# tangle-network/zk-SaaS

Hardware: AMD Instinct MI355X
Metric: Groth16 proofs/sec (SHA-256 circuit) (higher is better)
Workload: dtype u32 limbs (256-bit Montgomery); 1 GPU; BASELINE configs[3]: full distributed Groth16 on the SHA-256 circuit, BN254, l=2, n=8 parties on one GPU, all 12 masks sampled and applied (sha256.rs:226-291); masks=True, constraints=30006, wires=29823, domain=32768, len_a=14911, len_w=14911, len_u=16384, parties=8, packing_factor=2, fixed_base_tables=True

## Files before the change

zk-saas_amd/csrc/engine_groth16.inc.hpp:

```cpp

  int king3(const Fr* in, const zk_groth16_masks* mk, int first, int log_m, int inverse, const void* g, int scale,
            int rearrange, uint64_t seed, Fr* out, size_t per, hipStream_t st) {
    const Fr* U = nullptr;
    int rc = umat_for(nullptr, n, &U);
    if (rc) return rc;
    KingBatch<Fr> kb{};
    kb.stride = per;
    bool any = false, all = true;
    for (int k = 0; k < 3; k++) {
      kb.in_mask[k] = mk ? (const Fr*)mk->fft_in[first + k] : nullptr;
      kb.out_mask[k] = mk ? (const Fr*)mk->fft_out[first + k] : nullptr;
      any = any || kb.in_mask[k];
      all = all && kb.in_mask[k];
    }
    if (any == all)
      return king_dispatch_batch(in, kb, 3, n, log_m, inverse, U, g, scale, rearrange, seed, out, false, st);
    for (int k = 0; k < 3; k++) {
      rc = king_dispatch(in + k * per, kb.in_mask[k], n, log_m, inverse, U, g, scale, rearrange, seed + k,
                         out + k * per, kb.out_mask[k], false, st);
      if (rc) return rc;
    }
    return ZK_OK;
  }
  int circom_h(const void* qa, const void* qb, const void* qc, int log_m, const zk_groth16_masks* mk, uint64_t seed,
// ... 386 lines not shown
    ProveJob* J = &j;
    const size_t cstride = crs->len_a;
    const Fr* cf = msm_.coef_d_ + first;
    MsmGate gate{};
    const bool gated = j.gate_sorts = (full || gate_sorts) && log_m >= h_first_log_m_;
    j.sorted_cnt.store(0, std::memory_order_relaxed);
    if (gated) {
      gate.sorted_cnt = &j.sorted_cnt;
      gate.wait_sorted = j.ev_role;
      gate.n_wait_sorted = gate.sorted_need = 4;
    }
    auto role_gate = [&](MsmRole role) {
      MsmGate g = gate;
      if (g.n_wait_sorted) g.sorted_ev = J->ev_role[role];
      return g;
    };
    bool hu_done = false;
    if (full && gated) {
      hipError_t he = j.hshare.ensure((size_t)n * Lc * sizeof(Fr));
      if (he != hipSuccess) return hip_fail(he, "h share buffer");
      rc = circom_h_ws(qa, qb, qc, log_m, mk, seed, j.hshare.p, j.hwork, streams_[5]);
      if (rc) return rc;
      rc = msm_.template launch_t<Fq_>(this, j.ws0 + ROLE_U, crs->u_d, j.hshare.p, (size_t)n * crs->len_u,
                                      msm_.coef_d_, crs->len_u, streams_[5], &j.msm[ROLE_U], nullptr, u_gate(j));
      if (rc) return rc;
      hu_done = true;
    }
    msm_task<Fq2_>(j, ROLE_V, crs->v_d, nullptr, a_share, nullptr, (size_t)count * cstride, cf, cstride, streams_[2],
                   role_gate(ROLE_V), nullptr, [this, J](const P2* res) { take_V(*J, res); });
    const void* hd = j.pt.r_zero ? nullptr : crs->h_d;
    msm_task<Fq_>(j, ROLE_SH, crs->s_d, hd, a_share, nullptr, (size_t)count * cstride, cf, cstride, streams_[0],
                  role_gate(ROLE_SH), nullptr, [this, J, hd](const P1* res) { take_SH(*J, res, hd != nullptr); });
    msm_task<Fq_>(j, ROLE_W, crs->w_d, nullptr, ax_share, nullptr, (size_t)count * crs->len_w, cf, crs->len_w, streams_[3],
                  role_gate(ROLE_W), nullptr, [this, J](const P1* res) { take_W(*J, res); });
    if (!(full && !hu_done)) submit_host_terms(&j.pt, j.fut);
    if (full && !hu_done) {
      host_span(PROF_HOST_SUBMIT);
      hipStream_t hs = streams_[5];
      hipError_t he = j.hshare.ensure((size_t)n * Lc * sizeof(Fr));
      if (he != hipSuccess) return hip_fail(he, "h share buffer");
      rc = circom_h_ws(qa, qb, qc, log_m, mk, seed, j.hshare.p, j.hwork, hs);
      if (rc) return rc;
      host_span(PROF_HOST_H);
      rc = msm_.template launch_t<Fq_>(this, j.ws0 + ROLE_U, crs->u_d, j.hshare.p, (size_t)n * crs->len_u,
                                      msm_.coef_d_, crs->len_u, hs, &j.msm[ROLE_U]);
      if (rc) return rc;
      submit_host_terms(&j.pt, j.fut);
      host_span(PROF_HOST_U);
    }
    return ZK_OK;
  }

  void submit_host_terms(ProofTerms* J, std::vector<std::future<void>>& fut) {
    const bool full = J->full;
    const int first = J->first, count = J->count;
    if (full) {
      fut.push_back(pool_->submit([J]() {
        P1 d1 = aff1(J->crs.delta_g1);
        J->rN = host_scalar_mul<FrP, Fq_>(d1, J->r);
        J->s_cA = host_scalar_mul<FrP, Fq_>(xyzz_add_ni(xyzz_add_ni(aff1(J->crs.a_query0), J->rN), aff1(J->crs.alpha_g1)), J->s);
      }));
      fut.push_back(pool_->submit([J]() {
        P1 d1 = aff1(J->crs.delta_g1);
        J->sK = host_scalar_mul<FrP, Fq_>(d1, J->s);
        J->r_cB1 = host_scalar_mul<FrP, Fq_>(xyzz_add_ni(xyzz_add_ni(aff1(J->crs.b_g1_query0), J->sK), aff1(J->crs.beta_g1)), J->r);
      }));
      fut.push_back(pool_->submit([J]() { J->rsM = host_scalar_mul<FrP, Fq_>(aff1(J->crs.delta_g1), J->r * J->s); }));
      fut.push_back(pool_->submit([J]() { J->sK2 = host_scalar_mul<FrP, Fq2_>(aff2(J->crs.delta_g2), J->s); }));
// ... 10 lines not shown
            J->in1[k] = msm_.template mask_term<Fq_>(im, first, count);
            if (k == 0 && J->full) J->s_in0 = host_scalar_mul<FrP, Fq_>(J->in1[0], J->s);
            if (k == 1 && J->full) J->r_in1 = host_scalar_mul<FrP, Fq_>(J->in1[1], J->r);
          }
        }));
      }
      if (full)
        for (int p = 0; p < n; p++) {
          if (mk->msm_out[0])
            fut.push_back(pool_->submit([J, p]() {
              J->s_om0[p] = host_scalar_mul<FrP, Fq_>(jacobian_to_xyzz(((const Jacobian<Fq_>*)J->mk.msm_out[0])[p]), J->s);
            }));
          if (mk->msm_out[1] && !J->r_zero)
            fut.push_back(pool_->submit([J, p]() {
              J->r_om1[p] = host_scalar_mul<FrP, Fq_>(jacobian_to_xyzz(((const Jacobian<Fq_>*)J->mk.msm_out[1])[p]), J->r);
            }));
        }
    }
  }

  int prove_launch_u(ProveJob& j, const void* h_share, hipStream_t st) {
    const ProofTerms& t = j.pt;
    return msm_.template launch_t<Fq_>(this, j.ws0 + ROLE_U, t.crs.u_d, h_share, (size_t)t.count * t.crs.len_u,
                                      msm_.coef_d_ + t.first, t.crs.len_u, st, &j.msm[ROLE_U], nullptr, u_gate(j));
  }

  int prove_end(ProveJob& j, void* pi_a, void* pi_b, void* pi_c) {
    const char* who = "zk_groth16_wait";
    const auto t0 = std::chrono::steady_clock::now();
    int rc = drain_or_wedge(j, who);
    if (rc) return rc;
    bool early_ok = !j.pt.err.code;
    for (int e : j.rc) early_ok = early_ok && !e;
    std::vector<P1> c_part(early_ok ? n : 0);
    if (early_ok) assemble_job(j.pt, j.pt.sums(), pi_a, pi_b, pi_c, c_part.data());
    if (prof.on && job_slot(j, ROLE_U).busy) (void)event_wait(job_slot(j, ROLE_U).ev);
    const auto t2 = std::chrono::steady_clock::now();
    struct HostSpans {
      Profiler& pr;
      std::chrono::steady_clock::time_point a, b;
      ~HostSpans() {
        if (!pr.on) return;
        pr.host_add(PROF_HOST_WAIT, std::chrono::duration<double, std::milli>(b - a).count());
        pr.host_add(PROF_HOST_TAIL, std::chrono::duration<double, std::milli>(std::chrono::steady_clock::now() - b).count());
      }
    } spans{prof, t0, t2};
    rc = join(j, who);
// ... 335 lines not shown
```

zk-saas_amd/csrc/engine_points.inc.hpp:

```cpp

  int msm(int group, const void* bases, size_t nb, const void* scalars, size_t ns, void* out,
          hipStream_t st) override {
    if (nb != ns) {
      return fail(ZK_ERR_GENERIC, std::to_string(nb < ns ? nb : ns));
    }
    return msm_.run(this, group, bases, scalars, nb, out, st);
  }
  int d_msm(int group, const void* bases, const void* scalars, size_t len, const void* in_mask, const void* out_mask,
            void* out, hipStream_t st) override {
    return msm_.d_msm(this, group, bases, scalars, len, in_mask, out_mask, out, st);
  }

  static constexpr size_t BASE_MUL_WIDE_FROM = (size_t)1 << 19;
  template <class Fld>
  int base_mul_t(const void* base_affine, const void* scalars, size_t len, void* out_affine, hipStream_t st) {
    if (!len) return ZK_OK;
    if (!base_affine || !scalars || !out_affine) return fail(ZK_ERR_BAD_INPUT, "null pointer");
    const int nwin = (FrP::BITS + 7) / 8;
    std::string key((const char*)base_affine, sizeof(Affine<Fld>));
    Affine<Fld>* table = nullptr;
    {
      std::lock_guard<std::mutex> lk(mu_);
      auto it = base_tables_.find(key);
      if (it != base_tables_.end()) table = (Affine<Fld>*)it->second;
// ... 258 lines not shown
      if (value != 0 && (value < 8 || value > 22)) return fail(ZK_ERR_BAD_INPUT, "msm_table_c_g2 must be 0 (by length) or in 8..22");
      msm_.table_c_g2 = (int)value;
      return ZK_OK;
    }
    if (!strcmp(name, "wait_deadline_ms")) {
      if (value < 0 || value > 86400000) return fail(ZK_ERR_BAD_INPUT, "wait_deadline_ms must be in 0..86400000");
      wait_deadline_ms.store(value, std::memory_order_relaxed);
      return ZK_OK;
    }
    if (!strcmp(name, "host_threads")) {
      if (value < 0 || value > 256) return fail(ZK_ERR_BAD_INPUT, "host_threads must be in 0..256");
      if (value && value < 4) return fail(ZK_ERR_BAD_INPUT, "host_threads must be 0 (automatic) or at least 4");
      std::lock_guard<std::mutex> lk(mu_);
      if (streams_ready_) return fail(ZK_ERR_BAD_INPUT, "host_threads must be set before the first proof");
      host_threads_ = (int)value;
      return ZK_OK;
    }
    if (!strcmp(name, "msm_c") || !strcmp(name, "msm_c_g2")) {
      if (value != 0 && (value < 2 || value > 20)) return fail(ZK_ERR_BAD_INPUT, "msm_c must be 0 or in 2..20");
      if (name[5] == 0) msm_.c_g1 = msm_.c_g2 = (int)value;
      else msm_.c_g2 = (int)value;
      return ZK_OK;
    }
    if (!strcmp(name, "h_first_log_m")) {
      if (value < 1 || value > 64) return fail(ZK_ERR_BAD_INPUT, "h_first_log_m must be in 1..64");
      h_first_log_m_ = (int)value;
      return ZK_OK;
    }
    return fail(ZK_ERR_BAD_INPUT, "unknown option");
  }
  int msm_plan(int group, size_t len, int* plan) override {
    if (!plan || (group != ZK_G1 && group != ZK_G2)) return fail(ZK_ERR_BAD_INPUT, "bad argument");
    if (group == ZK_G2 && !Cfg::HAS_G2) return fail(ZK_ERR_BAD_INPUT, "G2 is not available for this curve");
    msm_.plan(len, group == ZK_G2, plan);
    return ZK_OK;
  }
  int group_add(int group, const void* a, const void* b, void* out) override {
    using Fq = Fp<typename Cfg::FqP>;
    using Fq2 = Fp2<typename Cfg::FqP>;
    if (!a || !b || !out) return fail(ZK_ERR_BAD_INPUT, "null pointer");
    if (group == ZK_G1) {
      Jacobian<Fq> x, y;
      memcpy(&x, a, sizeof(x));
      memcpy(&y, b, sizeof(y));
      Jacobian<Fq> o = xyzz_to_jacobian(xyzz_add_ni(jacobian_to_xyzz(x), jacobian_to_xyzz(y)));
      memcpy(out, &o, sizeof(o));
// ... 398 lines not shown
```

zk-saas_amd/csrc/msm.hpp:

```cpp
#pragma once
#include <algorithm>
#include <atomic>
#include <cstdio>
#include <cstdlib>
#include <future>
#include <map>
#include <memory>
#include <mutex>
#include <type_traits>
#include <vector>

#include "ec.hpp"
#include "engine.hpp"
#include "msm_plan.hpp"
#include "ntt.hpp"
#include "quad.hpp"

namespace zk {
#if defined(__HIPCC__)

enum MsmRole { ROLE_SH, ROLE_W, ROLE_V, ROLE_U, NROLES };
constexpr const char* ROLE_NAME[NROLES] = {"S+H", "W", "V", "U"};
constexpr int NJOBS = 2;
constexpr int NBATCH = 3;
// ... 1057 lines not shown
      for (uint32_t j = (uint32_t)vl; j < S; j += FIN_THREADS / 4) acc = qadd(acc, qload(hpart + vb + j, q), q);
      acc = wg_quad_sum(acc, sh, vl, q, FIN_THREADS / 4);
      if (vl == 0) qstore(buckets + heavy[2 + 2 * h], q, acc);
      __syncthreads();
    }
    return;
  }
  const uint32_t T = msm_range_len(offsets[nkeys], nlanes, tmin, cap);
  for (size_t k = (size_t)blockIdx.x * (FIN_THREADS / 4) + (threadIdx.x >> 2); k < nkeys;
       k += (size_t)fin_wgs * (FIN_THREADS / 4)) {
    const uint32_t o0 = offsets[k], o1 = offsets[k + 1];
    if (o0 == o1) {
      qstore(buckets + k, q, qidentity<Fld>(q));
      continue;
    }
    const uint32_t l0 = o0 / T, l1 = (o1 - 1) / T;
    if (l1 == l0 || l1 - l0 > FIN_SEQ) continue;
    Fld acc = qload(tail + l0, q);
    for (uint32_t l = l0 + 1; l <= l1; l++) acc = qadd(acc, qload(head + l, q), q);
    qstore(buckets + k, q, acc);
  }
}

template <class Fld>
__global__ __launch_bounds__(QUAD_THREADS, 2) void msm_reduce_a_kernel(const XYZZ<Fld>* __restrict__ buckets0, uint32_t B,
                                                                   int lo_bits, int nvl, XYZZ<Fld>* __restrict__ out0) {
  __builtin_amdgcn_s_setprio(3);
  extern __shared__ uint4 smem_red[];
  XYZZ<Fld>* sh = reinterpret_cast<XYZZ<Fld>*>(smem_red);
  const uint32_t LO = 1u << lo_bits, HI = B >> lo_bits;
  const uint32_t ngroups = HI + 1 + LO;
  const XYZZ<Fld>* __restrict__ wb = buckets0 + (size_t)blockIdx.y * B;
  const int q = threadIdx.x & 3, vl = threadIdx.x >> 2;
  const uint32_t g = blockIdx.x * (uint32_t)((int)blockDim.x / 4 / nvl) + (uint32_t)(vl / nvl);
  const uint32_t sub = (uint32_t)(vl & (nvl - 1));
  Fld acc = qidentity<Fld>(q);
  if (g <= HI) {
    for (uint32_t lo = sub; lo < LO; lo += (uint32_t)nvl) {
      uint32_t k = g * LO + lo;
      if (k >= 1 && k <= B) acc = qadd(acc, qload(wb + (k - 1), q), q);
    }
  } else if (g < ngroups) {
    const uint32_t lo = g - HI - 1;
    for (uint32_t hi = sub; hi <= HI; hi += (uint32_t)nvl) {
      uint32_t k = hi * LO + lo;
      if (k >= 1 && k <= B) acc = qadd(acc, qload(wb + (k - 1), q), q);
// ... 106 lines not shown
  const void* p[16] = {nullptr};
};

struct MsmPending {
  MsmFoldGeo fold;
  MsmSlot* slot = nullptr;
};

struct MsmGate {
  hipEvent_t sorted_ev = nullptr;
  std::atomic<int>* sorted_cnt = nullptr;
  const hipEvent_t* wait_sorted = nullptr;
  int n_wait_sorted = 0, sorted_need = 0;
  hipEvent_t wait_ev = nullptr;
  std::atomic<int>* wait_flag = nullptr;
  hipEvent_t signal_ev = nullptr;
  std::atomic<int>* signal_flag = nullptr;
};

struct MsmTuning {
  size_t bigsort_min;
  MsmGate gate;
  int c_force = 0;
};

template <class FrP, class Fld>
int msm_launch(IEngine* eng, MsmSlot& slot, const MsmTuning& tune, const void* bases, const void* bases2,
               const void* scalars, size_t npts, const Fp<FrP>* coef_d, size_t part_len, hipStream_t st,
               MsmPending* out, const MsmBatchArg* batch = nullptr);
template <class FrP, class Fld>
int pack_points_split_launch(IEngine* eng, const void* points, size_t nchunks, int n, const uint8_t* dig, int jlen,
                             const void* beta , void* shares, hipStream_t st);
template <class FrP, class Fld>
int base_mul_split_launch(IEngine* eng, const void* scalars, size_t len, const void* table, int nwin, int wb, void* out,
                          hipStream_t st);
template <class FrP, class Fld>
int msm_table_launch(IEngine* eng, const void* bases, size_t len, int c, int nwin, int wide, void* table,
                     hipStream_t st);

template <class Fld>
int msm_fold_batch(IEngine* eng, MsmPending& p, XYZZ<Fld>* results, int nvec) {
  const MsmFoldGeo& f = p.fold;
  const int batch = f.batch;
  for (int i = 0; i < nvec * batch; i++) results[i] = XYZZ<Fld>::identity();
  if (!p.slot) return ZK_OK;
  hipError_t he = p.slot->wait(eng);
// ... 124 lines not shown
  for (int nib = FrP::N * 8 - 1; nib >= 0; nib--) {
    for (int i = 0; i < 4; i++) acc = xyzz_dbl_ni(acc);
    for (int p = 0; p < np; p++) {
      uint32_t d = (k[p].v[nib / 8] >> (4 * (nib % 8))) & 15u;
      if (d) acc = xyzz_add_ni(acc, tab[(size_t)p * 15 + d - 1]);
    }
  }
  return acc;
}

template <class Cfg>
class MsmRunner {
 public:
  using FrP = typename Cfg::FrP;
  using Fr = Fp<FrP>;
  using Fq = Fp<typename Cfg::FqP>;
  using Fq2 = Fp2<typename Cfg::FqP>;

  void plan(size_t npts, bool g2, int* out) const {
    MsmPlanIn in;
    in.scalar_bits = FrP::BITS, in.scalar_bytes = (int)sizeof(Fr), in.coord_bytes = (int)(g2 ? sizeof(Fq2) : sizeof(Fq));
    in.g2 = g2, in.acc_waves = g2 ? SPLIT_WAVES<typename Cfg::FqP> : ACC_WAVES<Fq>;
    in.npts = npts, in.c_force = g2 ? c_g2 : c_g1, in.bigsort_min = bigsort_min;
    msm_plan_of(in, out);
  }
  int c_g1 = 0, c_g2 = 0;

  template <class Fld>
  int launch_t(IEngine* eng, int ws, const void* bases, const void* scalars, size_t npts, const Fr* coef_d,
               size_t part_len, hipStream_t st, MsmPending* pend, const void* bases2 = nullptr, MsmGate gate = MsmGate{},
               const MsmBatchArg* batch = nullptr) {
    if (ws < 0 || ws >= MSM_WS) return eng->fail(ZK_ERR_BAD_INPUT, "bad msm workspace slot");
    if (slots_[ws].busy) return eng->fail(ZK_ERR_GENERIC, "msm workspace slot still in flight");
    MsmTuning tune{bigsort_min, gate, IsExtField<Fld>::value ? c_g2 : c_g1};
    int rc = msm_launch<FrP, Fld>(eng, slots_[ws], tune, bases, bases2, scalars, npts, coef_d, part_len, st, pend,
                                  batch);
    if (rc) (void)slots_[ws].wait(eng);
    return rc;
  }
  template <class Fld, class Host>
  int run_t(IEngine* eng, int sid, const void* bases, const void* scalars, size_t npts, const Fr* coef_d,
            size_t part_len, hipStream_t st, XYZZ<Fld>* out, Host&& host, const MsmBatchArg* batch = nullptr) {
    int rc = eng->check_wedged();
    if (rc) return rc;
    std::unique_lock<std::mutex> lk(standalone_mu_, std::defer_lock);
    if (sid < 0) lk.lock();
    MsmPending pend;
    rc = launch_t<Fld>(eng, sid < 0 ? WS_STANDALONE : ws_dist(sid), bases, scalars, npts, coef_d, part_len, st, &pend,
                       nullptr, MsmGate{}, batch);
    if (!rc) {
      host();
      rc = msm_fold_batch<Fld>(eng, pend, out, 1);
    }
    if (rc && pend.slot && pend.slot->busy) {
      Status keep = eng->last;
      return eng->wedge(keep.msg);
    }
// ... 182 lines not shown
```

zk-saas_amd/csrc/msm_impl.hpp:

```cpp
#pragma once
#include "msm.hpp"
#include "pack_split.hpp"

namespace zk {

#define MSM_HIP(x)                                           \
  do {                                                       \
    hipError_t _e = (x);                                     \
    if (_e != hipSuccess) return eng->hip_fail(_e, #x);      \
  } while (0)
#ifdef ZK_MSM_DEBUG_SYNC
#define MSM_STAGE(name)                                                          \
  do {                                                                           \
    hipError_t _e = hipStreamSynchronize(st);                                    \
    fprintf(stderr, "[zk msm] %s done (%s) npts=%zu c=%d nwin=%d\n", name,       \
            hipGetErrorString(_e), pl.npts, pl.win.c, pl.win.nwin);              \
    if (_e != hipSuccess) return eng->hip_fail(_e, name);                        \
  } while (0)
#else
#define MSM_STAGE(name) do { } while (0)
#endif

template <class Fr, class KF>
struct MsmViews {
// ... 113 lines not shown
    msm_accumulate_split_kernel<typename BaseParams<Fld>::type><<<dim3((nlanes + 31) / 32, NB), dim3(128), 0, st>>>(
        bases, bases2, v.sorted, v.offsets, nkeys, nlanes, pl.tmin, pl.cap, v.buckets, v.edge, v.heavy, v.k0, pl.ys);
  } else {
    msm_accumulate_kernel<KF><<<dim3((nlanes + 127) / 128, NB), dim3(128), 0, st>>>(
        (const Affine<KF>*)bases, (const Affine<KF>*)bases2, v.sorted, v.offsets, nkeys, nlanes, pl.tmin, pl.cap, v.buckets,
        v.edge, v.heavy, v.k0, pl.ys, 0);
  }
  if (gate.signal_ev) {
    MSM_HIP(hipEventRecord(gate.signal_ev, st));
    if (gate.signal_flag) gate.signal_flag->store(1, std::memory_order_release);
  }
  return ZK_OK;
}

template <class Fr, class Fld, class KF>
int msm_stage_reduce(IEngine* eng, const MsmPlan& pl, const MsmViews<Fr, KF>& v, hipStream_t st) {
  constexpr bool G2FLD = IsExtField<Fld>::value;
  const unsigned NB = pl.vectors, nsets = (unsigned)pl.nsets;
  const uint32_t nkeys = (uint32_t)pl.nkeys, nlanes = pl.nlanes, tmin = pl.tmin, cap = pl.cap;
  const size_t ys = pl.ys;
  ProfScope ps_(eng->prof, G2FLD ? PROF_MSM_REDUCE_G2 : PROF_MSM_REDUCE, st, (double)pl.nkeys * NB);
  const int qt = quad_threads(pl.batch > 1), qvl = qt / 4;
  const size_t quad_lds = (size_t)qvl * sizeof(XYZZ<Fld>);
  msm_heavy_kernel<KF><<<dim3(2048, NB), dim3(64), (size_t)16 * sizeof(XYZZ<Fld>), st>>>(v.edge, nlanes, tmin, cap, v.offsets, nkeys,
                                                                    v.buckets, v.heavy, v.hpart, pl.vcap, ys);
  MSM_STAGE("heavy buckets");
  {
    const size_t fin_wgs = std::min<size_t>((pl.nkeys + FIN_THREADS / 4 - 1) / (FIN_THREADS / 4), 8192);
    const unsigned fin_extra = 256;
    msm_finalize_kernel<KF><<<dim3((unsigned)fin_wgs + fin_extra, NB), dim3(FIN_THREADS),
                              (size_t)(FIN_THREADS / 4) * sizeof(XYZZ<Fld>), st>>>(
        v.edge, nlanes, tmin, cap, v.offsets, nkeys, v.buckets, v.heavy, v.hpart, pl.vcap, (uint32_t)fin_wgs, ys);
  }
  MSM_STAGE("finalize");
  const size_t tot_groups = (size_t)pl.red_groups * NB * nsets;
  const size_t tot_slices = (size_t)pl.nslices * NB * nsets;
  const size_t cap_quads = (size_t)1024 * (G2FLD ? 2 : 3) * 16;
  auto pick_nvl = [&](size_t groups) {
    int n = qvl;
    while (n > 4 && groups * (size_t)n > cap_quads) n >>= 1;
    return n;
  };
  const int nvl_a = pick_nvl(tot_groups), nvl_b = pick_nvl(tot_slices);
  const unsigned gpw_a = (unsigned)(qvl / nvl_a), gpw_b = (unsigned)(qvl / nvl_b);
  msm_reduce_a_kernel<KF><<<dim3((pl.red_groups + gpw_a - 1) / gpw_a, NB * nsets), dim3((unsigned)qt), quad_lds, st>>>(
      v.buckets, pl.B, pl.lo_bits, nvl_a, v.rc);
  msm_reduce_b_kernel<KF><<<dim3(((unsigned)pl.nslices + gpw_b - 1) / gpw_b, NB * nsets), dim3((unsigned)qt), quad_lds, st>>>(
      v.rc, pl.B, pl.lo_bits, nvl_b, v.out,
      v.offsets + nkeys, ys, pl.nsorts, v.stats);
  return ZK_OK;
}

template <class FrP, class Fld>
int msm_launch(IEngine* eng, MsmSlot& slot, const MsmTuning& tune, const void* bases, const void* bases2,
               const void* scalars, size_t npts, const Fp<FrP>* coef_d, size_t part_len, hipStream_t st,
               MsmPending* pend, const MsmBatchArg* ba) {
  using Fr = Fp<FrP>;
// ... 2 lines not shown
  static_assert(sizeof(XYZZ<Fld>) == 4 * sizeof(Fld), "the plan sizes XYZZ points as four coordinates");
  constexpr bool G2FLD = IsExtField<Fld>::value;
  *pend = MsmPending{};
  const unsigned NB = bases2 ? 2u : 1u;
  const void* const bases_in = bases;
  const void* const bases2_in = bases2;
  size_t toff = 0, toff2 = 0;
  std::shared_ptr<const MsmTable> tab = TableRegistry::inst().find(bases, npts, sizeof(Affine<Fld>), FrP::BITS, &toff), tab2;
  if (tab && NB == 2) {
    tab2 = TableRegistry::inst().find(bases2, npts, sizeof(Affine<Fld>), FrP::BITS, &toff2);
    if (!tab2 || tab2->len != tab->len || toff2 != toff || tab2->c != tab->c) tab = nullptr;
    else bases2 = tab2->data;
  }
  if (tab) bases = tab->data;
  MsmPlanIn in;
  in.scalar_bits = FrP::BITS, in.scalar_bytes = (int)sizeof(Fr), in.coord_bytes = (int)sizeof(Fld), in.g2 = G2FLD;
  if constexpr (G2FLD) in.acc_waves = SPLIT_WAVES<typename BaseParams<Fld>::type>;
  else in.acc_waves = ACC_WAVES<Fld>;
  in.npts = npts, in.batch = ba ? (size_t)ba->nb : 1, in.vectors = (int)NB;
  if (tab) {
    in.tab_c = tab->c, in.tab_len = tab->len, in.tab_off = toff;
    in.tab_no_identity = !tab->any_identity && (NB == 1 || !tab2->any_identity);
  }
  in.c_force = tune.c_force, in.bigsort_min = tune.bigsort_min;
  const MsmPlan pl = msm_plan(in);
  if (pl.err) return eng->fail(ZK_ERR_BAD_INPUT, pl.err);
  pend->fold = pl.fold;
  if (npts == 0) return ZK_OK;
  hipError_t he = slot.ws.ensure(pl.ws_bytes);
  if (he != hipSuccess) return eng->hip_fail(he, "msm workspace");
  he = slot.ensure_pinned(pl.pinned_bytes);
  if (he != hipSuccess) return eng->hip_fail(he, "msm pinned buffer");
  if (!slot.ev) {
    he = hipEventCreateWithFlags(&slot.ev, hipEventDisableTiming);
    if (he != hipSuccess) return eng->hip_fail(he, "msm event");
  }
  slot.busy = true;
  slot.tab = tab;
  slot.tab2 = tab2;
  pend->slot = &slot;
  struct RecordOnExit {
    MsmSlot& s;
    hipStream_t st;
    bool done = false;
    ~RecordOnExit() {
      if (!done) (void)hipEventRecord(s.ev, st);
    }
// ... 87 lines not shown
```

zk-saas_amd/csrc/msm_plan.hpp:

```cpp
#pragma once
#include <algorithm>
#include <cstddef>
#include <cstdint>

namespace zk {

constexpr size_t MSM_RANGE_MIN = 20, MSM_RANGE = 64;
constexpr size_t MSM_RANGE_MIN_G2 = 16, MSM_RANGE_G2 = 64;
constexpr uint32_t FIN_SEQ = 16;
constexpr int MSM_MAXB = 16;

constexpr int BIG_HI = 8;
constexpr int BIG_MAX_BINS = 8192;
constexpr int BIG_THREADS = 256;
constexpr int BIG_PTS_PER_THREAD = 8;
constexpr int BIG_EPT = 16;
constexpr size_t BIG_LDS_MAX = 156 * 1024;
inline int msm_big_hi(size_t nsets) {
  int hi = BIG_HI;
  while (hi > 0 && (nsets << hi) > (size_t)BIG_MAX_BINS) hi--;
  return hi;
}
constexpr size_t msm_bins_words(size_t nbins) { return 3 * nbins + 2; }

constexpr int ISCAN_THREADS = 256;
constexpr int ISCAN_PER = 8;
constexpr int ISCAN_BLOCK = ISCAN_THREADS * ISCAN_PER;

inline size_t msm_heavy_cap(size_t nlanes) { return nlanes / FIN_SEQ + 8; }
inline size_t msm_heavy_vcap(size_t nlanes) { return nlanes / FIN_SEQ + nlanes / 256 + 8; }

struct MsmWindows {
// ... 9 lines not shown
  int width(int w) const { return w < wide ? c : c - 1; }
  int start(int w) const { return w * (c - 1) + std::min(w, wide); }
};

inline int msm_pick_c(int scalar_bits, size_t npts, int c_force = 0) {
  if (c_force >= 2 && c_force <= 20) return c_force;
  int best = 4;
  double best_cost = 1e300;
  for (int c = 4; c <= 20; c++) {
    int nwin = (scalar_bits + c) / c;
    int ceff = (scalar_bits + nwin) / nwin;
    double cost = (double)nwin * ((double)npts + (ceff > 17 ? 10.0 : 4.0) * (double)((size_t)1 << (ceff - 1)));
    if (cost <= best_cost) {
      best_cost = cost;
      best = c;
    }
  }
  return best;
}

struct MsmLanes {
  uint32_t nlanes, tmin, cap;
};
inline MsmLanes msm_pick_lanes(size_t max_entries, int waves, bool pair, int lanes_per_range = 0) {
  if (!lanes_per_range) lanes_per_range = pair ? 2 : 1;
  const size_t cap = (size_t)1024 * waves * (64 / lanes_per_range);
  const size_t lo = pair ? MSM_RANGE_MIN_G2 : MSM_RANGE_MIN;
  const size_t hi = pair ? MSM_RANGE_G2 : MSM_RANGE;
  size_t t = std::min(hi, std::max(lo, (size_t)((double)max_entries / (2.4 * (double)cap))));
  size_t nl = std::max<size_t>(1, (max_entries + t - 1) / t);
  if (max_entries >= cap * t && max_entries < 2 * cap * t && (max_entries + 2 * cap - 1) / (2 * cap) >= 12)
    nl = std::max(nl, 2 * cap);
  return MsmLanes{(uint32_t)nl, (uint32_t)t, (uint32_t)cap};
}

inline int table_c_auto(size_t len, bool g2) {
  if (g2) return len < ((size_t)1 << 20) ? 15 : 19;
  return len <= ((size_t)1 << 17) ? 15 : len < ((size_t)1 << 19) ? 16 : len < ((size_t)1 << 22) ? 18 : 20;
}

struct MsmFoldGeo {
  MsmWindows win;
  int kwin = 0;
  int lo_bits = 0;
  bool tabbed = false;
  int batch = 1;
  int nb = 1;
  int nsorts = 1;
  size_t stats_off = 0;
  size_t offered = 0;
  bool g2 = false;
};

struct MsmPlanIn {
  int scalar_bits = 0, scalar_bytes = 0;
  int coord_bytes = 0;
  bool g2 = false;
  int acc_waves = 0;
  size_t npts = 0, batch = 1;
  int vectors = 1;
  int tab_c = 0;
  size_t tab_len = 0, tab_off = 0;
  bool tab_no_identity = false;
  int c_force = 0;
  size_t bigsort_min = 0;
};

enum MsmRegionId {
  R_COUNTS, R_HEAVY, R_BINS, R_CURSOR, R_OFFSETS, R_BT, R_SORTED, R_K0, R_CANON, R_TMP, R_TMP_LO, R_TCNT,
  R_EDGE, R_BUCKETS, R_HPART, R_RC,
  R_COUNT,
  R_SORT_END = R_EDGE
};
struct MsmRegion {
  size_t off = 0, bytes = 0;
};

struct MsmPlan {
  const char* err = nullptr;
  size_t npts = 0, batch = 1;
  unsigned vectors = 1;
  MsmWindows win;
  uint32_t B = 0;
  bool tabbed = false;
  int kwin = 0;
  size_t nsets = 0, nkeys = 0;
  size_t max_sorted = 0;
  uint32_t pre_stride = 0, pre_off = 0;
  uint32_t nlanes = 0, tmin = 0, cap = 0;
  uint32_t vcap = 0;
  int lo_bits = 0;
  uint32_t red_groups = 0;
  int nslices = 0;
  size_t iscan_blocks = 0;
  bool no_identity = false;
  unsigned nsorts = 1;
  bool big = false;
  bool large = false;
  int sthr = 0, ppt = 0;
  int sort_hi = 0, sort_lo = 0;
  int idx_bits = 0;
  bool wide_fmt = false;
  size_t nbl = 0;
  size_t nbins_tot = 0;
  size_t stage_cap = 0, tile_pts = 0, tiles_big = 0;
  int wgroup = 0;
  bool use_tcnt = false;
  int hist_ppt = 0;
  size_t hist_lds = 0, scatter_lds = 0, binsort_lds = 0;
  MsmRegion r[R_COUNT];
  size_t sort_region = 0;
  size_t ys = 0;
  size_t ws_bytes = 0;
// ... 3 lines not shown
  MsmFoldGeo fold;
};

inline MsmPlan msm_plan(const MsmPlanIn& in) {
  MsmPlan p;
  const size_t npts = in.npts, batch = in.batch;
  const unsigned NB = in.vectors == 2 ? 2u : 1u;
  const bool tab = in.tab_c != 0;
  p.npts = npts, p.batch = batch, p.vectors = NB, p.tabbed = tab;
  if (batch < 1 || batch > (size_t)MSM_MAXB) {
    p.err = "bad msm batch";
    return p;
  }
  p.fold.batch = (int)batch;
  const MsmWindows win = MsmWindows::of(in.scalar_bits, tab ? in.tab_c : msm_pick_c(in.scalar_bits, npts ? npts : 1, in.c_force));
  const int c = win.c, nwin = win.nwin;
  p.win = win;
  p.B = 1u << (c - 1);
  const uint32_t B = p.B;
  const int kwin = p.kwin = tab ? 1 : nwin;
  const size_t nsets = p.nsets = batch * (size_t)kwin;
  const size_t nkeys = p.nkeys = nsets * B;
  const size_t max_sorted = p.max_sorted = npts * batch * nwin;
  const MsmLanes ml = msm_pick_lanes(max_sorted, in.acc_waves, in.g2, in.g2 ? 4 : 0);
  const uint32_t nlanes = p.nlanes = ml.nlanes;
  p.tmin = ml.tmin, p.cap = ml.cap;
  if (npts * batch >= ((size_t)1 << 31)) p.err = "msm too large";
  else if (max_sorted >= ((size_t)1 << 32)) p.err = "msm too large (points x windows >= 2^32)";
  if (p.err || !npts) return p;
  p.pre_stride = tab ? (uint32_t)in.tab_len : 0u, p.pre_off = tab ? (uint32_t)in.tab_off : 0u;
  p.vcap = (uint32_t)msm_heavy_vcap(nlanes);
  const int lo_bits = p.lo_bits = c / 2;
  p.red_groups = (B >> lo_bits) + 1 + (1u << lo_bits);
  p.nslices = c;
  p.iscan_blocks = (nkeys + ISCAN_BLOCK - 1) / ISCAN_BLOCK;
  p.no_identity = tab && in.tab_no_identity;
  const unsigned NS = p.nsorts = (NB == 2 && !p.no_identity) ? 2u : 1u;

  constexpr size_t large_min = (size_t)4 << 20;
  const bool large = p.large = npts * batch >= large_min;
  const int sthr = p.sthr = large ? 1024 : 256;
  int ppt = large ? BIG_PTS_PER_THREAD : 16;
  if (!large)
    while (ppt > 1 && ((npts + (size_t)sthr * ppt - 1) / ((size_t)sthr * ppt)) * batch < 1024) ppt >>= 1;
  const size_t stage_max = 16384;
  if (large && tab)
    while (ppt > 1 && (size_t)nwin * sthr * ppt > stage_max) ppt >>= 1;
  p.ppt = ppt;
  int sort_hi = std::min(msm_big_hi(nsets), std::max(1, c - 1 - 7));
  if (large) {
    auto lg = [](size_t v) { int l = 0; while (((size_t)1 << (l + 1)) <= v) l++; return l; };
    const int tp_eff = lg((size_t)sthr * ppt * (tab ? nwin : 1)), ch = lg((size_t)sthr * BIG_EPT);
    sort_hi = (c - 1 + tp_eff - ch + 1) / 2;
    if (sort_hi > c - 2) sort_hi = c - 2;
// ... 19 lines not shown
  const size_t tile_pts = p.tile_pts = (size_t)sthr * ppt;
  const bool big = p.big = npts * batch >= in.bigsort_min && sort_hi >= 1 && sort_lo >= 1 && sort_lo <= 12 &&
                           (nsets << sort_hi) <= (size_t)BIG_MAX_BINS &&
                           (large ? stage_cap >= (tab ? (size_t)nwin * tile_pts : tile_pts) : 8 * nbl <= BIG_LDS_MAX);
  p.wgroup = tab ? nwin : (int)std::min<size_t>((size_t)nwin, std::max<size_t>(1, stage_cap / tile_pts));
  const size_t nbins_tot = p.nbins_tot = nsets << sort_hi;
  p.tiles_big = ((npts + tile_pts - 1) / tile_pts) * batch;
  p.use_tcnt = big && large && tile_pts % BIG_THREADS == 0 && tile_pts < 65536;
  if (big) {
    p.hist_ppt = p.use_tcnt ? (int)(tile_pts / BIG_THREADS) : ppt;
    p.hist_lds = (nbins_tot + BIG_THREADS / 64) * 4;
    p.scatter_lds = large ? (2 * nbl + (size_t)(sthr / 64)) * 4 + stage_cap * (wide_fmt ? 8 : 6) : 2 * nbl * 4;
    p.binsort_lds = (2 * ((size_t)1 << sort_lo) + 1 + (size_t)(sthr / 64)) * 4 + (large ? (size_t)sthr * BIG_EPT * 6 : 0);
  }

  size_t off = 0;
  auto take = [&](MsmRegionId id, size_t bytes) {
    p.r[id].off = off;
    p.r[id].bytes = bytes;
    off += (bytes + 255) & ~(size_t)255;
  };
  const size_t xyzz = 4 * (size_t)in.coord_bytes;
  take(R_COUNTS, nkeys * 4);
  take(R_HEAVY, msm_heavy_cap(nlanes) * 8 + 16);
  take(R_BINS, big ? msm_bins_words(nbins_tot) * 4 : 0);
  p.zero_off = big ? p.r[R_HEAVY].off : p.r[R_COUNTS].off;
  p.zero_bytes = big ? p.r[R_BINS].off + (nbins_tot + 1) * 4 - p.zero_off : p.r[R_HEAVY].off + 16 - p.zero_off;
  take(R_CURSOR, nkeys * 4);
  take(R_OFFSETS, (nkeys + 1) * 4);
  take(R_BT, p.iscan_blocks * 4);
  take(R_SORTED, max_sorted * 4);
  take(R_K0, (size_t)nlanes * 4);
  take(R_CANON, npts * batch * (size_t)in.scalar_bytes);
  if (big) {
    take(R_TMP, max_sorted * 4);
    if (wide_fmt) take(R_TMP_LO, max_sorted * 2);
    if (p.use_tcnt) take(R_TCNT, p.tiles_big * nbl * 2);
  }
  p.sort_region = off;
  p.ys = NS == 2 ? p.sort_region : 0;
  off = p.sort_region * NS;
  take(R_EDGE, NB * 2 * (size_t)nlanes * xyzz);
  take(R_BUCKETS, NB * nkeys * xyzz);
  take(R_HPART, NB * (size_t)p.vcap * xyzz);
  take(R_RC, NB * nsets * p.red_groups * xyzz);
  p.ws_bytes = off;
  p.out_bytes = NB * nsets * p.nslices * xyzz;
  p.pinned_bytes = p.out_bytes + 64;

  p.fold.win = win;
// ... 22 lines not shown
```

zk-saas_amd/csrc/quad.hpp:

```cpp
#pragma once
#include "ec.hpp"
#include "ntt.hpp"

namespace zk {
#if defined(__HIPCC__)

template <int P0, int P1, int P2, int P3>
ZK_D uint32_t qperm_u32(uint32_t v) {
  return (uint32_t)__builtin_amdgcn_mov_dpp((int)v, P0 | (P1 << 2) | (P2 << 4) | (P3 << 6), 0xf, 0xf, true);
}
template <int P0, int P1, int P2, int P3, class P>
ZK_D Fp<P> qperm(const Fp<P>& v) {
  Fp<P> r;
#pragma unroll
  for (int i = 0; i < P::N; i++) r.v[i] = qperm_u32<P0, P1, P2, P3>(v.v[i]);
  return r;
}
template <int P0, int P1, int P2, int P3, class P, bool I>
ZK_D Fp2T<P, I> qperm(const Fp2T<P, I>& v) {
  return {qperm<P0, P1, P2, P3>(v.c0), qperm<P0, P1, P2, P3>(v.c1)};
}
template <class P>
ZK_D Fp<P> qsel(bool a, const Fp<P>& x, const Fp<P>& y) {
  Fp<P> r;
#pragma unroll
  for (int i = 0; i < P::N; i++) r.v[i] = a ? x.v[i] : y.v[i];
  return r;
}
template <class P, bool I>
ZK_D Fp2T<P, I> qsel(bool a, const Fp2T<P, I>& x, const Fp2T<P, I>& y) {
  return {qsel(a, x.c0, y.c0), qsel(a, x.c1, y.c1)};
}

template <class Fld>
ZK_D Fld qidentity(int q) {
  return q < 2 ? Fld::one() : Fld::zero();
}
template <class Fld>
ZK_D Fld qload(const XYZZ<Fld>* p, int q) {
  return load_elem(reinterpret_cast<const Fld*>(p) + q);
}
template <class Fld>
ZK_D void qstore(XYZZ<Fld>* p, int q, const Fld& c) {
  store_elem(reinterpret_cast<Fld*>(p) + q, c);
}

template <class Fld>
ZK_D Fld qadd(const Fld& ca, const Fld& cb, int q) {
  const bool even = (q & 1) == 0;
  const bool za = qperm<2, 2, 2, 2>(ca).is_zero();
  const bool zb = qperm<2, 2, 2, 2>(cb).is_zero();
  Fld A = qsel(even, qperm<0, 0, 1, 1>(ca), qperm<0, 0, 1, 1>(cb));
  Fld B = qsel(even, qperm<2, 2, 3, 3>(cb), qperm<2, 2, 3, 3>(ca));
  const Fld m1 = A * B;
  const Fld d = qperm<1, 1, 3, 3>(m1) - qperm<0, 0, 2, 2>(m1);
  const bool pz = qperm<0, 0, 0, 0>(d).is_zero();
  const bool rz = qperm<2, 2, 2, 2>(d).is_zero();
  const bool D = pz && rz && !za && !zb;
  const Fld cu = qsel(q == 1, ca.dbl(), ca);
  A = qsel(D, cu, qsel(even, d, qperm<0, 2, 2, 3>(ca)));
  B = qsel(D, cu, qsel(even, d, qperm<0, 2, 2, 3>(cb)));
  const Fld m2 = A * B;
  const Fld XX = qperm<0, 0, 0, 0>(m2);
  const Fld M = XX.dbl() + XX;
  A = qsel(D, qsel(q == 3, M, cu), qsel(q == 2, qperm<0, 1, 1, 3>(m2), qsel(q == 1, d, m1)));
  B = qsel(D, qsel(q == 3, M, qperm<1, 1, 1, 1>(m2)), XX);
  const Fld m3 = A * B;
// ... 189 lines not shown
```

Before: 636.1 proofs/s.

## Fuse heavy-bucket and finalize MSM stages into one tail kernel for U MSM

Adds a fused msm_tail_kernel that handles heavy buckets (split across workgroups, with an atomic ticket so the last one combines the partials) and light-bucket finalization in a single launch. Light buckets are combined with a DPP row-rotate tree over groups of four lanes. The fused kernel is enabled for the U (h) MSM launches, which sit at the end of the dependency chain, and can be forced for all MSMs through a new 'msm_tail_latency' option. It targets a kernel launch and a serial stage on the critical path, at the cost of extra ticket memory that must be zeroed and a more complex synchronisation scheme.

```diff
diff --git a/zk-saas_amd/csrc/engine_groth16.inc.hpp b/zk-saas_amd/csrc/engine_groth16.inc.hpp
--- a/zk-saas_amd/csrc/engine_groth16.inc.hpp
+++ b/zk-saas_amd/csrc/engine_groth16.inc.hpp
@@ -432,7 +432,8 @@
       rc = circom_h_ws(qa, qb, qc, log_m, mk, seed, j.hshare.p, j.hwork, streams_[5]);
       if (rc) return rc;
       rc = msm_.template launch_t<Fq_>(this, j.ws0 + ROLE_U, crs->u_d, j.hshare.p, (size_t)n * crs->len_u,
-                                      msm_.coef_d_, crs->len_u, streams_[5], &j.msm[ROLE_U], nullptr, u_gate(j));
+                                      msm_.coef_d_, crs->len_u, streams_[5], &j.msm[ROLE_U], nullptr, u_gate(j), nullptr,
+                                      true );
       if (rc) return rc;
       hu_done = true;
     }
@@ -453,7 +454,8 @@
       if (rc) return rc;
       host_span(PROF_HOST_H);
       rc = msm_.template launch_t<Fq_>(this, j.ws0 + ROLE_U, crs->u_d, j.hshare.p, (size_t)n * crs->len_u,
-                                      msm_.coef_d_, crs->len_u, hs, &j.msm[ROLE_U]);
+                                      msm_.coef_d_, crs->len_u, hs, &j.msm[ROLE_U], nullptr, MsmGate{}, nullptr,
+                                      true );
       if (rc) return rc;
       submit_host_terms(&j.pt, j.fut);
       host_span(PROF_HOST_U);
@@ -510,7 +512,8 @@
   int prove_launch_u(ProveJob& j, const void* h_share, hipStream_t st) {
     const ProofTerms& t = j.pt;
     return msm_.template launch_t<Fq_>(this, j.ws0 + ROLE_U, t.crs.u_d, h_share, (size_t)t.count * t.crs.len_u,
-                                      msm_.coef_d_ + t.first, t.crs.len_u, st, &j.msm[ROLE_U], nullptr, u_gate(j));
+                                      msm_.coef_d_ + t.first, t.crs.len_u, st, &j.msm[ROLE_U], nullptr, u_gate(j), nullptr,
+                                      true );
   }
 
   int prove_end(ProveJob& j, void* pi_a, void* pi_b, void* pi_c) {
diff --git a/zk-saas_amd/csrc/engine_points.inc.hpp b/zk-saas_amd/csrc/engine_points.inc.hpp
--- a/zk-saas_amd/csrc/engine_points.inc.hpp
+++ b/zk-saas_amd/csrc/engine_points.inc.hpp
@@ -304,6 +304,11 @@
       else msm_.c_g2 = (int)value;
       return ZK_OK;
     }
+    if (!strcmp(name, "msm_tail_latency")) {
+      if (value != 0 && value != 1) return fail(ZK_ERR_BAD_INPUT, "msm_tail_latency must be 0 or 1");
+      msm_.tail_latency = (int)value;
+      return ZK_OK;
+    }
     if (!strcmp(name, "h_first_log_m")) {
       if (value < 1 || value > 64) return fail(ZK_ERR_BAD_INPUT, "h_first_log_m must be in 1..64");
       h_first_log_m_ = (int)value;
diff --git a/zk-saas_amd/csrc/msm.hpp b/zk-saas_amd/csrc/msm.hpp
--- a/zk-saas_amd/csrc/msm.hpp
+++ b/zk-saas_amd/csrc/msm.hpp
@@ -1103,6 +1103,103 @@
   }
 }
 
+constexpr uint32_t FIN_TREE_PRE = 2;
+template <class Fld>
+constexpr int TAIL_WAVES = sizeof(Fld) <= 32 ? 4 : sizeof(Fld) <= 48 ? 3 : 2;
+template <class Fld>
+__global__ __launch_bounds__(FIN_THREADS, TAIL_WAVES<Fld>) void msm_tail_kernel(const XYZZ<Fld>* __restrict__ edge0, uint32_t nlanes,
+                                                               uint32_t tmin, uint32_t cap,
+                                                               const uint32_t* __restrict__ offsets, uint32_t nkeys,
+                                                               XYZZ<Fld>* __restrict__ buckets0, uint32_t* __restrict__ heavy,
+                                                               XYZZ<Fld>* __restrict__ hpart0, uint32_t vcap, uint32_t hcap,
+                                                               uint32_t heavy_wgs, size_t ys) {
+  static_assert(FIN_TREE_G == 4 && FIN_THREADS == 64, "a group is one DPP row: 16 lanes, four per wave");
+  __builtin_amdgcn_s_setprio(3);
+  ZK_YSHIFT(offsets);
+  const XYZZ<Fld>* __restrict__ head = edge0 + (size_t)blockIdx.y * 2 * nlanes;
+  const XYZZ<Fld>* __restrict__ tail = head + nlanes;
+  XYZZ<Fld>* __restrict__ buckets = buckets0 + (size_t)blockIdx.y * nkeys;
+  const int q = threadIdx.x & 3, vl = threadIdx.x >> 2;
+  if (blockIdx.x < heavy_wgs) {
+    ZK_YSHIFT(heavy);
+    const uint32_t nh = heavy[1], V = heavy[0];
+    if (blockIdx.x >= V) return;
+    uint32_t* ticket = heavy + 2 + 2 * (size_t)hcap + (ys ? 0 : (size_t)blockIdx.y * hcap);
+    XYZZ<Fld>* hpart = hpart0 + (size_t)blockIdx.y * vcap;
+    extern __shared__ uint4 smem_fin[];
+    XYZZ<Fld>* sh = reinterpret_cast<XYZZ<Fld>*>(smem_fin);
+    __shared__ uint32_t last_sh;
+    constexpr int nq = FIN_THREADS / 4;
+    const uint32_t T = msm_range_len(offsets[nkeys], nlanes, tmin, cap);
+    for (uint32_t v = blockIdx.x; v < V; v += heavy_wgs) {
+      uint32_t lo = 0, hi = nh;
+      while (hi - lo > 1) {
+        const uint32_t mid = (lo + hi) >> 1;
+        if (heavy[3 + 2 * mid] <= v) lo = mid;
+        else hi = mid;
+      }
+      const uint32_t kh = heavy[2 + 2 * lo], vb = heavy[3 + 2 * lo];
+      const uint32_t S = (lo + 1 < nh ? heavy[3 + 2 * (lo + 1)] : V) - vb, s = v - vb;
+      const uint32_t o0 = offsets[kh], o1 = offsets[kh + 1];
+      const uint32_t l0 = o0 / T, l1 = (o1 - 1) / T;
+      const uint32_t chunk = (l1 - l0 + S - 1) / S;
+      const uint32_t first = l0 + 1 + s * chunk, last = first + chunk - 1 < l1 ? first + chunk - 1 : l1;
+      Fld acc = (s == 0 && vl == 0) ? qload(tail + l0, q) : qidentity<Fld>(q);
+      for (uint32_t l = first + (uint32_t)vl; l <= last; l += (uint32_t)nq) acc = qadd(acc, qload(head + l, q), q);
+      acc = wg_quad_sum(acc, sh, vl, q, nq);
+      if (vl == 0) qstore(S == 1 ? buckets + kh : hpart + v, q, acc);
+      if (S > 1) {
+        __builtin_amdgcn_fence(__ATOMIC_RELEASE, "agent");
+        __syncthreads();
+        if (threadIdx.x == 0)
+          last_sh = __hip_atomic_fetch_add(ticket + lo, 1u, __ATOMIC_ACQ_REL, __HIP_MEMORY_SCOPE_AGENT) == S - 1 ? 1u : 0u;
+        __syncthreads();
+        if (last_sh) {
+          __builtin_amdgcn_fence(__ATOMIC_ACQUIRE, "agent");
+          Fld t = qidentity<Fld>(q);
+          for (uint32_t j = (uint32_t)vl; j < S; j += (uint32_t)nq) t = qadd(t, qload_agent(hpart + vb + j, q), q);
+          t = wg_quad_sum(t, sh, vl, q, nq);
+          if (vl == 0) qstore(buckets + kh, q, t);
+        }
+      }
+      __syncthreads();
+    }
+    return;
+  }
+  const uint32_t T = msm_range_len(offsets[nkeys], nlanes, tmin, cap);
+  const uint32_t fin_wgs = gridDim.x - heavy_wgs;
+  constexpr uint32_t GPW = FIN_THREADS / 4 / FIN_TREE_G;
+  const uint32_t j = (uint32_t)vl & (FIN_TREE_G - 1);
+  for (size_t k = (size_t)(blockIdx.x - heavy_wgs) * GPW + (uint32_t)vl / FIN_TREE_G; k < nkeys; k += (size_t)fin_wgs * GPW) {
+    const uint32_t o0 = offsets[k], o1 = offsets[k + 1];
+    if (o0 == o1) {
+      if (j == 0) qstore(buckets + k, q, qidentity<Fld>(q));
+      continue;
+    }
+    const uint32_t l0 = o0 / T, l1 = (o1 - 1) / T;
+    if (l1 == l0 || l1 - l0 > FIN_SEQ) continue;
+    const uint32_t n = l1 - l0 + 1;
+    auto slot = [&](uint32_t i) {
+      const uint32_t idx = j + i * FIN_TREE_G, ic = idx < n ? idx : n - 1;
+      return qsel(idx < n, qload(ic ? head + l0 + ic : tail + l0, q), qidentity<Fld>(q));
+    };
+    Fld p[FIN_TREE_PRE];
+#pragma unroll
+    for (uint32_t i = 0; i < FIN_TREE_PRE; i++) p[i] = slot(i);
+    const uint32_t trips = (n + FIN_TREE_G - 1) / FIN_TREE_G;
+    Fld acc = p[0];
+#pragma unroll 1
+    for (uint32_t it = 1; it < trips + 2; it++) {
+      const Fld other = qsel(it < trips, p[1], qsel(it == trips, qrow_ror<8>(acc), qrow_ror<4>(acc)));
+#pragma unroll
+      for (uint32_t i = 1; i + 1 < FIN_TREE_PRE; i++) p[i] = p[i + 1];
+      p[FIN_TREE_PRE - 1] = slot(it + FIN_TREE_PRE - 1);
+      acc = qadd(acc, other, q);
+    }
+    if (j == 0) qstore(buckets + k, q, acc);
+  }
+}
+
 template <class Fld>
 __global__ __launch_bounds__(QUAD_THREADS, 2) void msm_reduce_a_kernel(const XYZZ<Fld>* __restrict__ buckets0, uint32_t B,
                                                                    int lo_bits, int nvl, XYZZ<Fld>* __restrict__ out0) {
@@ -1255,6 +1352,7 @@
   size_t bigsort_min;
   MsmGate gate;
   int c_force = 0;
+  bool chain_end = false;
 };
 
 template <class FrP, class Fld>
@@ -1425,17 +1523,19 @@
     in.scalar_bits = FrP::BITS, in.scalar_bytes = (int)sizeof(Fr), in.coord_bytes = (int)(g2 ? sizeof(Fq2) : sizeof(Fq));
     in.g2 = g2, in.acc_waves = g2 ? SPLIT_WAVES<typename Cfg::FqP> : ACC_WAVES<Fq>;
     in.npts = npts, in.c_force = g2 ? c_g2 : c_g1, in.bigsort_min = bigsort_min;
+    in.chain_end = tail_latency != 0;
     msm_plan_of(in, out);
   }
   int c_g1 = 0, c_g2 = 0;
+  int tail_latency = 0;
 
   template <class Fld>
   int launch_t(IEngine* eng, int ws, const void* bases, const void* scalars, size_t npts, const Fr* coef_d,
                size_t part_len, hipStream_t st, MsmPending* pend, const void* bases2 = nullptr, MsmGate gate = MsmGate{},
-               const MsmBatchArg* batch = nullptr) {
+               const MsmBatchArg* batch = nullptr, bool chain_end = false) {
     if (ws < 0 || ws >= MSM_WS) return eng->fail(ZK_ERR_BAD_INPUT, "bad msm workspace slot");
     if (slots_[ws].busy) return eng->fail(ZK_ERR_GENERIC, "msm workspace slot still in flight");
-    MsmTuning tune{bigsort_min, gate, IsExtField<Fld>::value ? c_g2 : c_g1};
+    MsmTuning tune{bigsort_min, gate, IsExtField<Fld>::value ? c_g2 : c_g1, chain_end || tail_latency != 0};
     int rc = msm_launch<FrP, Fld>(eng, slots_[ws], tune, bases, bases2, scalars, npts, coef_d, part_len, st, pend,
                                   batch);
     if (rc) (void)slots_[ws].wait(eng);
diff --git a/zk-saas_amd/csrc/msm_impl.hpp b/zk-saas_amd/csrc/msm_impl.hpp
--- a/zk-saas_amd/csrc/msm_impl.hpp
+++ b/zk-saas_amd/csrc/msm_impl.hpp
@@ -159,17 +159,27 @@
   ProfScope ps_(eng->prof, G2FLD ? PROF_MSM_REDUCE_G2 : PROF_MSM_REDUCE, st, (double)pl.nkeys * NB);
   const int qt = quad_threads(pl.batch > 1), qvl = qt / 4;
   const size_t quad_lds = (size_t)qvl * sizeof(XYZZ<Fld>);
-  msm_heavy_kernel<KF><<<dim3(2048, NB), dim3(64), (size_t)16 * sizeof(XYZZ<Fld>), st>>>(v.edge, nlanes, tmin, cap, v.offsets, nkeys,
-                                                                    v.buckets, v.heavy, v.hpart, pl.vcap, ys);
-  MSM_STAGE("heavy buckets");
-  {
-    const size_t fin_wgs = std::min<size_t>((pl.nkeys + FIN_THREADS / 4 - 1) / (FIN_THREADS / 4), 8192);
-    const unsigned fin_extra = 256;
-    msm_finalize_kernel<KF><<<dim3((unsigned)fin_wgs + fin_extra, NB), dim3(FIN_THREADS),
-                              (size_t)(FIN_THREADS / 4) * sizeof(XYZZ<Fld>), st>>>(
-        v.edge, nlanes, tmin, cap, v.offsets, nkeys, v.buckets, v.heavy, v.hpart, pl.vcap, (uint32_t)fin_wgs, ys);
-  }
-  MSM_STAGE("finalize");
+  if (pl.chain_end) {
+    const size_t gpw = FIN_THREADS / 4 / FIN_TREE_G;
+    const size_t fin_wgs = std::min<size_t>((pl.nkeys + gpw - 1) / gpw, (size_t)1024 * TAIL_WAVES<KF>);
+    const unsigned heavy_wgs = 512;
+    msm_tail_kernel<KF><<<dim3(heavy_wgs + (unsigned)fin_wgs, NB), dim3(FIN_THREADS), (size_t)(FIN_THREADS / 4) * sizeof(XYZZ<Fld>),
+                          st>>>(v.edge, nlanes, tmin, cap, v.offsets, nkeys, v.buckets, v.heavy, v.hpart, pl.vcap, pl.hcap,
+                                heavy_wgs, ys);
+    MSM_STAGE("tail");
+  } else {
+    msm_heavy_kernel<KF><<<dim3(2048, NB), dim3(64), (size_t)16 * sizeof(XYZZ<Fld>), st>>>(v.edge, nlanes, tmin, cap, v.offsets, nkeys,
+                                                                      v.buckets, v.heavy, v.hpart, pl.vcap, ys);
+    MSM_STAGE("heavy buckets");
+    {
+      const size_t fin_wgs = std::min<size_t>((pl.nkeys + FIN_THREADS / 4 - 1) / (FIN_THREADS / 4), 8192);
+      const unsigned fin_extra = 256;
+      msm_finalize_kernel<KF><<<dim3((unsigned)fin_wgs + fin_extra, NB), dim3(FIN_THREADS),
+                                (size_t)(FIN_THREADS / 4) * sizeof(XYZZ<Fld>), st>>>(
+          v.edge, nlanes, tmin, cap, v.offsets, nkeys, v.buckets, v.heavy, v.hpart, pl.vcap, (uint32_t)fin_wgs, ys);
+    }
+    MSM_STAGE("finalize");
+  }
   const size_t tot_groups = (size_t)pl.red_groups * NB * nsets;
   const size_t tot_slices = (size_t)pl.nslices * NB * nsets;
   const size_t cap_quads = (size_t)1024 * (G2FLD ? 2 : 3) * 16;
@@ -218,7 +228,7 @@
     in.tab_c = tab->c, in.tab_len = tab->len, in.tab_off = toff;
     in.tab_no_identity = !tab->any_identity && (NB == 1 || !tab2->any_identity);
   }
-  in.c_force = tune.c_force, in.bigsort_min = tune.bigsort_min;
+  in.c_force = tune.c_force, in.bigsort_min = tune.bigsort_min, in.chain_end = tune.chain_end;
   const MsmPlan pl = msm_plan(in);
   if (pl.err) return eng->fail(ZK_ERR_BAD_INPUT, pl.err);
   pend->fold = pl.fold;
diff --git a/zk-saas_amd/csrc/msm_plan.hpp b/zk-saas_amd/csrc/msm_plan.hpp
--- a/zk-saas_amd/csrc/msm_plan.hpp
+++ b/zk-saas_amd/csrc/msm_plan.hpp
@@ -8,6 +8,9 @@
 constexpr size_t MSM_RANGE_MIN = 20, MSM_RANGE = 64;
 constexpr size_t MSM_RANGE_MIN_G2 = 16, MSM_RANGE_G2 = 64;
 constexpr uint32_t FIN_SEQ = 16;
+constexpr uint32_t FIN_TREE_G = 4;
+constexpr uint32_t FIN_TREE_SLOTS = (FIN_SEQ + 1 + FIN_TREE_G - 1) / FIN_TREE_G;
+constexpr size_t MSM_RANGE_MIN_CHAIN_END = 20;
 constexpr int MSM_MAXB = 16;
 
 constexpr int BIG_HI = 8;
@@ -63,10 +66,10 @@
 struct MsmLanes {
   uint32_t nlanes, tmin, cap;
 };
-inline MsmLanes msm_pick_lanes(size_t max_entries, int waves, bool pair, int lanes_per_range = 0) {
+inline MsmLanes msm_pick_lanes(size_t max_entries, int waves, bool pair, int lanes_per_range = 0, size_t lo_chain_end = 0) {
   if (!lanes_per_range) lanes_per_range = pair ? 2 : 1;
   const size_t cap = (size_t)1024 * waves * (64 / lanes_per_range);
-  const size_t lo = pair ? MSM_RANGE_MIN_G2 : MSM_RANGE_MIN;
+  const size_t lo = lo_chain_end ? lo_chain_end : pair ? MSM_RANGE_MIN_G2 : MSM_RANGE_MIN;
   const size_t hi = pair ? MSM_RANGE_G2 : MSM_RANGE;
   size_t t = std::min(hi, std::max(lo, (size_t)((double)max_entries / (2.4 * (double)cap))));
   size_t nl = std::max<size_t>(1, (max_entries + t - 1) / t);
@@ -105,6 +108,7 @@
   bool tab_no_identity = false;
   int c_force = 0;
   size_t bigsort_min = 0;
+  bool chain_end = false;
 };
 
 enum MsmRegionId {
@@ -130,6 +134,8 @@
   uint32_t pre_stride = 0, pre_off = 0;
   uint32_t nlanes = 0, tmin = 0, cap = 0;
   uint32_t vcap = 0;
+  bool chain_end = false;
+  uint32_t hcap = 0;
   int lo_bits = 0;
   uint32_t red_groups = 0;
   int nslices = 0;
@@ -179,7 +185,9 @@
   const size_t nsets = p.nsets = batch * (size_t)kwin;
   const size_t nkeys = p.nkeys = nsets * B;
   const size_t max_sorted = p.max_sorted = npts * batch * nwin;
-  const MsmLanes ml = msm_pick_lanes(max_sorted, in.acc_waves, in.g2, in.g2 ? 4 : 0);
+  p.chain_end = in.chain_end;
+  const MsmLanes ml = msm_pick_lanes(max_sorted, in.acc_waves, in.g2, in.g2 ? 4 : 0,
+                                     in.chain_end && !in.g2 ? MSM_RANGE_MIN_CHAIN_END : 0);
   const uint32_t nlanes = p.nlanes = ml.nlanes;
   p.tmin = ml.tmin, p.cap = ml.cap;
   if (npts * batch >= ((size_t)1 << 31)) p.err = "msm too large";
@@ -187,6 +195,7 @@
   if (p.err || !npts) return p;
   p.pre_stride = tab ? (uint32_t)in.tab_len : 0u, p.pre_off = tab ? (uint32_t)in.tab_off : 0u;
   p.vcap = (uint32_t)msm_heavy_vcap(nlanes);
+  p.hcap = (uint32_t)msm_heavy_cap(nlanes);
   const int lo_bits = p.lo_bits = c / 2;
   p.red_groups = (B >> lo_bits) + 1 + (1u << lo_bits);
   p.nslices = c;
@@ -252,10 +261,11 @@
   };
   const size_t xyzz = 4 * (size_t)in.coord_bytes;
   take(R_COUNTS, nkeys * 4);
-  take(R_HEAVY, msm_heavy_cap(nlanes) * 8 + 16);
+  take(R_HEAVY, (size_t)p.hcap * (in.chain_end ? 16 : 8) + 16);
   take(R_BINS, big ? msm_bins_words(nbins_tot) * 4 : 0);
   p.zero_off = big ? p.r[R_HEAVY].off : p.r[R_COUNTS].off;
-  p.zero_bytes = big ? p.r[R_BINS].off + (nbins_tot + 1) * 4 - p.zero_off : p.r[R_HEAVY].off + 16 - p.zero_off;
+  p.zero_bytes = big ? p.r[R_BINS].off + (nbins_tot + 1) * 4 - p.zero_off
+                     : p.r[R_HEAVY].off + (in.chain_end ? p.r[R_HEAVY].bytes : 16) - p.zero_off;
   take(R_CURSOR, nkeys * 4);
   take(R_OFFSETS, (nkeys + 1) * 4);
   take(R_BT, p.iscan_blocks * 4);
diff --git a/zk-saas_amd/csrc/quad.hpp b/zk-saas_amd/csrc/quad.hpp
--- a/zk-saas_amd/csrc/quad.hpp
+++ b/zk-saas_amd/csrc/quad.hpp
@@ -20,6 +20,18 @@
 ZK_D Fp2T<P, I> qperm(const Fp2T<P, I>& v) {
   return {qperm<P0, P1, P2, P3>(v.c0), qperm<P0, P1, P2, P3>(v.c1)};
 }
+template <int N, class P>
+ZK_D Fp<P> qrow_ror(const Fp<P>& v) {
+  static_assert(N % 4 == 0 && N > 0 && N < 16, "whole quads");
+  Fp<P> r;
+#pragma unroll
+  for (int i = 0; i < P::N; i++) r.v[i] = (uint32_t)__builtin_amdgcn_mov_dpp((int)v.v[i], 0x120 + N, 0xf, 0xf, true);
+  return r;
+}
+template <int N, class P, bool I>
+ZK_D Fp2T<P, I> qrow_ror(const Fp2T<P, I>& v) {
+  return {qrow_ror<N>(v.c0), qrow_ror<N>(v.c1)};
+}
 template <class P>
 ZK_D Fp<P> qsel(bool a, const Fp<P>& x, const Fp<P>& y) {
   Fp<P> r;
@@ -43,6 +55,18 @@
 template <class Fld>
 ZK_D void qstore(XYZZ<Fld>* p, int q, const Fld& c) {
   store_elem(reinterpret_cast<Fld*>(p) + q, c);
+}
+
+template <class Fld>
+ZK_D Fld qload_agent(const XYZZ<Fld>* p, int q) {
+  static_assert(sizeof(Fld) % 4 == 0, "whole words");
+  const uint32_t* s = reinterpret_cast<const uint32_t*>(reinterpret_cast<const Fld*>(p) + q);
+  uint32_t w[sizeof(Fld) / 4];
+#pragma unroll
+  for (size_t i = 0; i < sizeof(Fld) / 4; i++) w[i] = __hip_atomic_load(s + i, __ATOMIC_RELAXED, __HIP_MEMORY_SCOPE_AGENT);
+  Fld r;
+  __builtin_memcpy(&r, w, sizeof(Fld));
+  return r;
 }
 
 template <class Fld>
```

Result: no change. 631.7 proofs/s (-0.7%).
